# pathint/RankCompV3.jl

Measured on AMD Instinct MI355X. Metric: gene-pair·sample comparisons/sec at 20k genes × 1k samples, higher is better.
Workload: dtype u16

## Files before the change

rankcompv3.jl_amd/_ffi.py:

```python
from __future__ import annotations

import ctypes
import os
import subprocess
from typing import NamedTuple

import numpy as np

_HERE = os.path.dirname(os.path.abspath(__file__))
LIB_PATH = os.environ.get("REO_LIB_PATH") or os.path.join(_HERE, "libreo_hip.so")
CSRC = os.path.join(_HERE, "csrc")

REO_OK, REO_EINVAL, REO_EHIP, REO_ECOMM, REO_ENOMEM = 0, -1, -2, -3, -4
NTIMINGS = 12
CALL_BINS = 8192

SYMBOLS = [
    "reo_version", "reo_last_error", "reo_create", "reo_destroy", "reo_trim_memory", "reo_set_shard", "reo_set_allreduce", "reo_set_allgather",
    "reo_create_multi", "reo_comm_unique_id", "reo_comm_init_rank",
    "reo_set_matrix_f64", "reo_set_matrix_i64", "reo_set_matrix_dev_f64", "reo_set_matrix_dev_i64",
    "reo_set_matrix_f32", "reo_set_matrix_i32", "reo_set_matrix_dev_f32", "reo_set_matrix_dev_i32",
    "reo_set_matrix_rm_f64", "reo_set_matrix_rm_i64", "reo_set_matrix_rm_f32", "reo_set_matrix_rm_i32",
    "reo_set_matrix_csc_f64", "reo_set_matrix_csc_i64", "reo_set_matrix_csc_f32", "reo_set_matrix_csc_i32",
    "reo_set_groups", "reo_compute_thresholds", "reo_set_thresholds", "reo_get_thresholds", "reo_threshold",
# ... 837 lines not shown
    def get_matrix(self) -> np.ndarray:
        info = self.info()
        dt = {1: np.float64, 2: np.int64, 3: np.float32}.get(info["resident_dtype"])
        if dt is None:
            raise DimensionMismatch(REO_EINVAL, "no expression matrix set")
        out = np.zeros((info["G"], info["S"]), dtype=dt, order="F")
        check(self._L.reo_get_matrix(self._h, _ptr(out), out.nbytes))
        return out

    def set_profiling(self, on: bool) -> None:
        check(self._L.reo_set_profiling(self._h, 1 if on else 0))

    def reset_timings(self) -> None:
        check(self._L.reo_reset_timings(self._h))

    def timings(self) -> dict:
        ms = np.zeros(NTIMINGS, dtype=np.float64)
        check(self._L.reo_get_timings(self._h, _ptr(ms), NTIMINGS))
        return {"transform_ms": ms[0], "k1_ms": ms[1], "k2_ms": ms[2], "iter_ms": ms[3], "k3_ms": max(ms[3] - ms[2], 0.0), "k2_launches": int(ms[4]),
                "k1_launches": int(ms[5]), "exchange_ms": ms[6], "pseudobulk_ms": ms[7], "k2_full_ms": ms[8],
                "k2_full_launches": int(ms[9]), "k2_delta_ms": ms[10], "set_matrix_host_wall_ms": ms[11]}

    def info(self) -> dict:
        w = np.zeros(32, dtype=np.int64)
        check(self._L.reo_get_info(self._h, _ptr(w), 32))
        v = np.zeros(28, dtype=np.int64)
        v[:] = w[:28]
        return {"G": int(v[0]), "S": int(v[1]), "Gp": int(v[2]), "table_bytes": int(v[3]), "has_ties": int(v[4]),
                "tiles_owned": int(v[5]), "tiles_total": int(v[6]), "tile_i": int(v[7]), "chunk_j": int(v[8]),
                "chunks_per_panel": int(v[9]), "unit_h": int(v[10]), "sample_slots": int(v[11]),
                "shared_group_counts": int(v[12]), "group_count_bytes": int(v[13]), "transform_in_lds": int(v[14]), "xcc_local_histograms": int(v[15]),
                "cycle_period": int(v[16]), "cycle_found_at_pass": int(v[17]), "cycle_passes_skipped": int(v[18]), "upload_link_bytes": int(v[19]),
                "eager_range_launches": int(v[20]), "rowmajor_upload": int(v[21]),
                "csc_upload": int(v[22]), "csc_nnz": int(v[23]), "resident_dtype": int(v[24]),
                "k1_slot_order": int(v[25]), "k1_half_tiles_separated": int(v[26]), "csc_device": int(v[27]),
                "k1_unslot_form": int(w[28]), "contrast_treat": int(w[29]), "k1_slot_sides": int(w[30]),
                "masked_build": int(w[31])}
```

rankcompv3.jl_amd/csrc/api.hip:

```cpp
#include <execinfo.h>
#include <signal.h>
#include <unistd.h>

#include <ctime>
#include <algorithm>
#include <chrono>
#include <cmath>
#include <cstdarg>
#include <cstdio>
#include <cstdlib>
#include <cstring>

#include "reo_internal.h"
#include "contrast.h"
#include "masked_pairs.h"
#include "sample_counts.h"
#include "upload_csc.h"

#include <mutex>
#include <unordered_map>

namespace reo {

static thread_local std::string g_err;
// ... 217 lines not shown
    (void)!write(2, head, sizeof head - 1);
    void *frames[64];
    const int n = backtrace(frames, 64);
    backtrace_symbols_fd(frames, n, 2);
    sigaction(sig, &g_old_action[sig == SIGSEGV ? 0 : (sig == SIGBUS ? 1 : 2)], nullptr);
    raise(sig);
}

static void install_segv_backtrace()
{
    static bool done = false;
    if (done) return;
    done = true;
    void *warm[2];
    (void)backtrace(warm, 2);
    struct sigaction sa;
    memset(&sa, 0, sizeof sa);
    sa.sa_handler = segv_backtrace;
    sa.sa_flags = SA_NODEFER;
    sigaction(SIGSEGV, &sa, &g_old_action[0]);
    sigaction(SIGBUS, &sa, &g_old_action[1]);
    sigaction(SIGABRT, &sa, &g_old_action[2]);
}

static double wall_us()
{
    timespec ts;
    clock_gettime(CLOCK_MONOTONIC, &ts);
    return ts.tv_sec * 1e6 + ts.tv_nsec * 1e-3;
}

static void drop_ref_mask(reo_ctx *c, const char *why)
{
    c->ref_slot = -1;
    c->ref_gone = why;
}

int32_t wait_or_drop_table(reo_ctx *c)
{
    const hipError_t e = stream_wait(c);
    if (e == hipSuccess) return REO_OK;
    c->built_k = -1;
    c->table_complete = false;
    drop_ref_mask(c, "a kernel queued on this context failed and the class table was dropped");
    set_error("a kernel queued on this context failed: %s (the class table was dropped: call reo_build_pairs again)", hipGetErrorString(e));
    return REO_EHIP;
// ... 246 lines not shown
    c->sc_slot2col_uploaded = nullptr;
    REO_HIP_CHECK(hipMemcpyAsync(c->sc_slot2col.p, c->sc_slot2col_host.data(), map.size() * sizeof(int32_t), hipMemcpyHostToDevice, c->stream));
    c->sc_slot2col_uploaded = c->sc_slot2col.p;
    return REO_OK;
}

int32_t need_complete_table(reo_ctx *c)
{
    if (c->built_k < 0) { set_error("no class table: call reo_build_pairs first"); return REO_EINVAL; }
    if (!c->table_complete) {
        set_error("shard %d of %d holds only its own part of the class table: attach a communicator (reo_comm_init_rank) or an "
                  "exchange hook (reo_set_allgather, reo_set_allreduce) before reo_build_pairs", c->rank, c->world);
        return REO_ECOMM;
    }
    return REO_OK;
}

}

using namespace reo;

extern "C" {

int32_t reo_version(void) { return 1200; }

int32_t reo_trim_memory(void)
{
    std::vector<Block> all;
    {
        Pool &P = pool();
        std::lock_guard<std::mutex> lk(P.mu);
        all.swap(P.free_blocks);
        P.cached = 0;
    }
    int dev = 0;
    const bool have_dev = hipGetDevice(&dev) == hipSuccess;
    for (const Block &b : all) {
        if (!b.pinned) (void)hipSetDevice(b.device);
        raw_free(b.p, b.pinned);
    }
    {
        Handles &H = handles();
        std::lock_guard<std::mutex> lk(H.mu);
        for (int k = 0; k < 2; ++k) {
            for (auto &st : H.streams[k]) { (void)hipSetDevice(st.first); (void)hipStreamDestroy(st.second); }
            for (auto &ev : H.events[k]) { (void)hipSetDevice(ev.first); (void)hipEventDestroy(ev.second); }
            H.streams[k].clear(); H.events[k].clear();
// ... 31 lines not shown
    if (const char *e = getenv("REO_K1_WAVE")) c->k1_wave = (e[0] != '0');
    if (const char *e = getenv("REO_K1_HALF")) c->k1_half = (e[0] != '0');
    if (const char *e = getenv("REO_K1_SLOTS")) c->k1_slots = (e[0] != '0');
    if (const char *e = getenv("REO_K1_QUEUE")) c->k1_queue = (e[0] != '0');
    if (const char *e = getenv("REO_K1_UNSLOT")) { const int v = atoi(e); c->k1_unslot = (v == 8 || v == 4) ? v : (e[0] == '0' ? 0 : -1); }
    if (const char *e = getenv("REO_K1_SLOT_SIDES")) { const int v = atoi(e); c->k1_slot_sides = (v == 1 || v == 2) ? v : 0; }
    if (const char *e = getenv("REO_K1_WORKERS")) c->k1_workers = std::max(1, atoi(e));
    if (const char *e = getenv("REO_K1_ORDER")) c->k1_order = std::max(0, std::min(2, atoi(e)));
    {
        int n = 0;
        if (hipDeviceGetAttribute(&n, hipDeviceAttributeMultiprocessorCount, c->device) == hipSuccess && n > 0) c->n_cus = n;
    }
    if (const char *e = getenv("REO_SPIN_WAIT")) c->spin_wait = (e[0] != '0');
    if (const char *e = getenv("REO_CHECK_HOOK_TABLE")) c->check_hook_table = (e[0] != '0');
    if (const char *e = getenv("REO_SHARE_GROUP_COUNTS")) c->share_counts = (e[0] != '0');
    if (const char *e = getenv("REO_LIGHT_BAND")) c->light_band = std::max(0, atoi(e));
    if (const char *e = getenv("REO_HIST_BELOW")) c->hist_below = std::max(0, atoi(e));
    if (const char *e = getenv("REO_CYCLE")) c->cycle_watch = atoi(e) != 0;
    if (const char *e = getenv("REO_LIGHT")) c->light_mode = e[0] == '0' ? 0 : (e[0] == '2' ? 2 : (e[0] == '3' ? 3 : 1));
    c->light_window = light_window(); c->light_min_g = light_min_genes();
    if (const char *e = getenv("REO_LIGHT_WINDOW")) c->light_window = std::max(1, std::min(31, atoi(e)));
    if (const char *e = getenv("REO_LIGHT_MIN_G")) c->light_min_g = std::max(64, atoi(e));
    if (const char *e = getenv("REO_STATE_MIRROR")) c->state_mirror_wanted = (e[0] != '0');
    if (const char *e = getenv("REO_EXCHANGE_WAVES")) c->x_waves = std::max(1, std::min(8, atoi(e)));
    if (const char *e = getenv("REO_EAGER_UPLOAD")) c->eager_mode = std::max(0, std::min(2, atoi(e)));
    if (const char *e = getenv("REO_EAGER_CHUNK")) c->eager_chunk = std::max(1, atoi(e));
    if (const char *e = getenv("REO_EAGER_GATE")) c->eager_gate = atoi(e) != 0;
    if (const char *e = getenv("REO_EAGER_RANGES")) c->eager_ranges = std::max(1, std::min(6, atoi(e)));
    if (const char *e = getenv("REO_UPLOAD_THREADS")) c->upload_threads = std::max(0, std::min(64, atoi(e)));
    c->debug_passes = getenv("REO_DEBUG_PASSES") != nullptr;
    c->debug_stamps = getenv("REO_DEBUG_STAMPS") != nullptr;
    c->k1_stamps = getenv("REO_K1_STAMPS") != nullptr;
    hipError_t e = handle_stream(&c->stream, 0);
    if (e != hipSuccess) { delete c; set_error("hipStreamCreate failed: %s", hipGetErrorString(e)); return REO_EHIP; }
    int ok = 0;
    const char *xe = getenv("REO_XCC_LOCAL");
    if (!(xe && xe[0] == '0')) {
        const int32_t rc = xcc_selftest(c, &ok);
        if (rc) { reo_destroy(c); return rc; }
    }
    c->xcc_local = ok;
    *out = c;
    return REO_OK;
}

void reo_destroy(reo_ctx *c)
// ... 23 lines not shown
    for (auto &e : c->ev_rk) release_event(e, 0);
    for (auto &e : c->ev_up) release_event(e, 0);
    c->e_lists.release();
    for (int q = 0; q < 3; ++q) {
        if (c->stage_h[q]) pool_free(c->stage_h[q], c->stage_cap, true);
        c->stage_d[q].release();
        release_event(c->ev_stage[q], 0);
        release_event(c->ev_widen[q], 0);
    }
    release_event(c->ev_fork, 0);
    release_event(c->ev_x, 0);
    for (auto &e : c->ev_k1) release_event(e, 0);
    c->t_pos16.release(); c->t_lo16.release(); c->t_hi16.release(); c->gcounts.release();
    c->k1_slot_part.release(); c->k1_slot_maps.release(); c->pos_s.release(); c->lo_s.release(); c->k1_queue_ctr.release();
    c->t_pos32.release(); c->t_lo32.release(); c->t_hi32.release(); c->t_vin32.release(); c->t_vout32.release();
    for (int t = 0; t < 2; ++t) { c->refbits[t].release(); c->refbytes[t].release(); }
    c->raw.release(); c->delta_list.release(); c->cont.release(); c->result.release(); c->sorted_d.release(); c->sorted_p.release();
    c->rank_s.release(); c->rank_a.release(); c->scal.release(); c->blockmin.release();
    c->state.release(); c->trace.release(); c->modes.release(); c->cand.release(); c->hist.release(); c->mrank.release(); c->lstate.release(); c->clist.release(); c->olist.release(); c->units_all.release(); c->xsend.release(); c->xrecv.release(); c->check_flag.release(); c->gridbar.release(); c->chunk_v.release(); c->chunk_i.release(); c->part.release();
    if (c->host_state) pool_free(c->host_state, sizeof(IterState), true);
    if (c->host_flags) pool_free(c->host_flags, 8 * sizeof(int32_t), true);
    release_event(c->ev_flags, 0);
    if (c->host_ref) pool_free(c->host_ref, c->host_ref_cap, true);
    release_stream(c->stream, 0);
    delete c;
    tl_release_synced = false;
}

int32_t reo_set_shard(reo_ctx *c, int32_t rank, int32_t world)
{
    if (!c) { set_error("null context"); return REO_EINVAL; }
    if (world < 1 || rank < 0 || rank >= world) { set_error("bad shard %d of %d", rank, world); return REO_EINVAL; }
    if (!c->peers.empty()) { set_error("a multi-GPU context (reo_create_multi) shards by itself"); return REO_EINVAL; }
    c->rank = rank; c->world = world;
    c->built_k = -1;
    drop_ref_mask(c, "reo_set_shard dropped the class table that the last reo_identify_degs ran on");
    c->eager_k1 = false;
    c->gc_valid = false;
    c->table_complete = false;
    return REO_OK;
}

int32_t reo_set_allreduce(reo_ctx *c, reo_allreduce_fn fn, void *user)
{
    if (!c) { set_error("null context"); return REO_EINVAL; }
    c->ar = fn; c->ar_user = user;
// ... 573 lines not shown
        st.need_full = 1;
        st.raw_pass = -1;
        st.kstar = -1;
        st.cyc_period = -1;
        *c->host_state = st;
    }
    const bool watch = c->cycle_watch && c->light_mode != 0 && (c->light_mode == 1 || G > 65535) && G >= c->light_min_g && n_iter > 0;
    if (watch) {
        if ((rc = c->snap.ensure(2 * static_cast<size_t>(c->Gp)))) return rc;
        c->host_state->cyc_period = 0;
    }
    c->it_cycle_period = 0; c->it_cycle_at = 0; c->it_cycle_skipped = 0;
    DrainOnExit drain(c);
    if ((rc = launch_iter_init(c, c->host_ref, c->host_state))) return rc;
    c->it_pval_deg = pval_deg; c->it_padj_deg = padj_deg; c->it_n_iter = n_iter; c->it_n_conv = n_conv;
    c->it_a0 = static_cast<int>(a - 1); c->it_b0 = static_cast<int>(b - 1);
    c->k2_idx = 0;
    const int light_form = (G > 65535 && c->light_mode != 0) ? 1 : c->light_mode;
    c->it_light_form = light_form;
    c->state_mirror = light_form != 2 && c->state_mirror_wanted;
    bool small = G < c->light_min_g || c->light_mode == 0;
    c->it_no_light = false;
    int passes = 0, seen_need_full = 1, light_batches = 0, idle_light = 0, idle_any = 0;
    while (n_iter > 0) {
        const int remaining = n_iter - passes;
        const double w_loop = c->debug_passes ? wall_us() : 0.0;
        const int nfull = small ? std::min(8, remaining) : (seen_need_full ? std::min(passes == 0 ? 4 : 2, remaining) : 0);
        const int nlight = (small || seen_need_full) ? 0 : std::min(light_batches == 0 ? 32 : kLightBatch, remaining);
        if (nlight > 0) ++light_batches;
        tic(c, 3);
        for (int t = 0; t < nfull; ++t)
            if ((rc = launch_full_pass(c, false))) return rc;
        if (nlight > 0 && light_form == 2) {
            if ((rc = launch_light_persistent(c))) return rc;
        } else if (nlight > 0) {
            if ((rc = launch_light_batch(c, nlight))) return rc;
        }
        toc(c);
        if (!c->state_mirror) REO_HIP_CHECK(hipMemcpyAsync(c->host_state, c->state.p, sizeof(IterState), hipMemcpyDeviceToHost, c->stream));
        const double w0 = c->debug_passes ? wall_us() : 0.0;
        if ((rc = wait_or_drop_table(c))) return rc;
        if (c->debug_passes) fprintf(stderr, "  waited %.0f us for the batch (enqueueing it took %.0f us)\n", wall_us() - w0, w0 - w_loop);
        if (c->debug_passes && nlight > 0 && light_form == 3) {
            static LightState hs;
            if (hipMemcpy(&hs, c->lstate.p, sizeof hs, hipMemcpyDeviceToHost) == hipSuccess)
                for (int q = 1; q <= nlight; ++q)
                    if (hs.slot[q].pad0[0] || q <= 3)
                        fprintf(stderr, "  launch %d: why %d (1 window, 2 se left the bracket, 4 the histogram's cut left the band, 8 a list overflowed, 16 too many listed, 32 cut below the band), "
                                "cut of the m_lo histogram %d, listed %d, surely inside %d, cut %d (band around %d), eta %.3g, se %.10g\n", q, hs.slot[q].pad0[0], hs.slot[q].pad0[1],
                                hs.slot[q].pad0[2], hs.slot[q].pad0[3], hs.slot[q].pad0[4], hs.slot[q - 1].rec.kstar, hs.slot[q - 1].eta, hs.slot[q].se_base);
        }
        if (c->debug_passes)
            fprintf(stderr, "batch: %d sorting + %d light launches, passes %d -> %d, need_full %d, done %d, last_full %d, changed genes in front of the next pass %d\n", nfull, nlight,
                    passes, c->host_state->passes, c->host_state->need_full, c->host_state->done, c->host_state->last_full,
                    c->host_state->delta_cnt[c->host_state->passes & 1]);
        if ((rc = pass_fault(c))) return rc;
        idle_any = c->host_state->passes == passes ? idle_any + 1 : 0;
        if (idle_any >= 4) {
            set_error("the iteration made no progress in four batches of launches (passes %d, need_full %d): loop control fault", passes, c->host_state->need_full);
            return REO_EHIP;
        }
        if (nlight > 0) idle_light = c->host_state->passes == passes ? idle_light + 1 : 0;
        if (idle_light >= 2 && !small) {
            small = true;
            c->it_no_light = true;
        }
        if (c->host_state->passes < passes || c->host_state->passes > n_iter) {
            set_error("the iteration's pass counter reads %d after %d of %d passes: loop control fault", c->host_state->passes, passes, n_iter);
            return REO_EHIP;
        }
        passes = c->host_state->passes;
        seen_need_full = c->host_state->need_full;
        if (c->host_state->done || passes >= n_iter) break;
        if (c->host_state->cyc_period > 0) {
            const int p = c->host_state->cyc_period, P = (p & 1) ? 2 * p : p;
            const int skip = (n_iter - passes - 1) / P * P;
            if ((rc = launch_cycle_skip(c, skip, p))) return rc;
            c->it_cycle_period = p; c->it_cycle_at = passes; c->it_cycle_skipped = skip;
            if (c->debug_passes) fprintf(stderr, "cycle: the reference set in front of pass %d equals that of pass %d; %d passes skipped\n", passes, passes - p, skip);
            passes += skip;
        }
    }
    if (passes > 0 && !c->host_state->last_full) {
        tic(c, 3);
        if ((rc = launch_full_pass(c, true))) return rc;
        toc(c);
    }
    if (trace && passes > 0)
        REO_HIP_CHECK(hipMemcpyAsync(trace, c->trace.p, sizeof(int32_t) * 2 * passes, hipMemcpyDeviceToHost, c->stream));
    const int nk2 = std::min<int>(c->k2_idx, static_cast<int>(c->modes.n));
    if (c->profiling && nk2 > 0) {
        c->k2_modes.assign(c->k2_idx, 0);
        REO_HIP_CHECK(hipMemcpyAsync(c->k2_modes.data(), c->modes.p, sizeof(int32_t) * nk2, hipMemcpyDeviceToHost, c->stream));
    }
    if (c->debug_stamps) {
        unsigned long long st[24];
        REO_HIP_CHECK(hipMemcpy(st, c->scal.p + 32, sizeof st, hipMemcpyDeviceToHost));
        if (light_form == 3) {
            fprintf(stderr, "stamps kl_one (inputs back, se, cut, lists + mask step, changed rows, delta1, sums + windows, end):");
            for (int k = 0; k <= 7; ++k) fprintf(stderr, " %lld", (long long)(st[k] - st[8]));
        } else if (light_form == 2) {
            fprintf(stderr, "stamps kl_persist, one pass (phase 1, barrier, phase 2, barrier, loads asked, cut, mask step):");
            for (int k = 1; k <= 7; ++k) fprintf(stderr, " %lld", (long long)(st[k] - st[0]));
        } else {
            fprintf(stderr, "stamps kl_head (inputs back, cut, mask step, changed rows, delta1, window flags, block sums, end):");
            for (int k = 0; k <= 7; ++k) fprintf(stderr, " %lld", (long long)(st[k] - st[8]));
            fprintf(stderr, "\nstamps kl_rank (inputs back, selection + se, p + BH rank, end):");
            for (int k = 20; k <= 23; ++k) fprintf(stderr, " %lld", (long long)(st[k] - st[19]));
        }
        fprintf(stderr, "  (x 10 ns)\n");
    }
    if (iters_run) *iters_run = passes;
    const double w_copy = c->debug_passes ? wall_us() : 0.0;
    REO_HIP_CHECK(hipMemcpyAsync(result, c->result.p, sizeof(double) * 15 * G, hipMemcpyDeviceToHost, c->stream));
    const double w_copied = c->debug_passes ? wall_us() : 0.0;
    if ((rc = wait_or_drop_table(c))) return rc;
    drain.dismiss();
    if (c->debug_passes) fprintf(stderr, "  result copy: enqueued in %.0f us, waited %.0f us\n", w_copied - w_copy, wall_us() - w_copied);
    collect_timings(c);
    if ((rc = pass_fault(c))) return rc;
    if (passes > 0) c->ref_slot = (passes - 1) & 1;
    else drop_ref_mask(c, "the last reo_identify_degs was called with n_iter <= 0: no pass ran, no tallies were counted");
    return REO_OK;
}

int32_t reo_get_ref_mask(reo_ctx *c, uint8_t *ref_mask, int32_t *nref)
{
    int32_t rc = use(c);
    if (rc) return rc;
    if (!ref_mask) { set_error("reo_get_ref_mask: ref_mask must not be null"); return REO_EINVAL; }
    if (c->ref_slot < 0 || c->built_k < 0) {
        set_error("reo_get_ref_mask: no reference set to deliver: %s", c->ref_slot < 0 ? c->ref_gone : "the class table was dropped");
        return REO_EINVAL;
    }
    DrainOnExit drain(c);
    REO_HIP_CHECK(hipMemcpyAsync(ref_mask, c->refbytes[c->ref_slot].p, static_cast<size_t>(c->G), hipMemcpyDeviceToHost, c->stream));
    REO_HIP_CHECK(hipStreamSynchronize(c->stream));
    drain.dismiss();
    int32_t n = 0;
    for (int64_t i = 0; i < c->G; ++i) { ref_mask[i] = ref_mask[i] != 0; n += ref_mask[i]; }
    if (nref) *nref = n;
// ... 34 lines not shown
{
    if (!c) { set_error("null context"); return REO_EINVAL; }
    collect_timings(c);
    for (double &v : c->t_ms) v = 0.0;
    return REO_OK;
}

int32_t reo_get_timings(reo_ctx *c, double *ms, int32_t n)
{
    if (!c || !ms) { set_error("null argument"); return REO_EINVAL; }
    collect_timings(c);
    for (int i = 0; i < n && i < REO_NTIMINGS; ++i) ms[i] = c->t_ms[i];
    return REO_OK;
}

int32_t reo_get_info(reo_ctx *c, int64_t *info, int32_t n)
{
    if (!c || !info) { set_error("null argument"); return REO_EINVAL; }
    int64_t separated = 0;
    if (n > 26 && c->last_k1_slots) {
        int32_t rc = use(c);
        if (rc || (rc = launch_slot_separated(c, &separated))) return rc;
    }
    const int64_t v[32] = {c->G, c->S, c->Gp, static_cast<int64_t>(c->table.n * sizeof(uint32_t)), c->has_ties,
                           c->tiles_owned, c->tiles_total, kTileI, c->k1_cj, c->k1_q, kUnitH,
                           c->goff32.empty() ? 0 : c->goff32.back(), c->last_k1_shared,
                           static_cast<int64_t>(c->gcounts.n * sizeof(uint16_t)), c->transform_in_lds, c->xcc_local,
                           c->it_cycle_period, c->it_cycle_at, c->it_cycle_skipped, c->narrowed_bytes, c->eager_range_launches, c->rowmajor_upload,
                           c->csc_upload, c->csc_nnz, c->dtype, c->last_k1_slots, separated, c->csc_device,
                           c->last_k1_slots ? c->last_k1_unslot : 0, c->built_k >= 0 ? c->built_treat : -1,
                           c->last_k1_slots ? c->last_k1_slot_sides : 0, (c->built_k >= 0 && c->built_masked) ? 1 : 0};
    for (int i = 0; i < n && i < 32; ++i) info[i] = v[i];
    return REO_OK;
}

}
```

rankcompv3.jl_amd/csrc/kernels.hip:

```cpp
#include <algorithm>
#include <chrono>
#include <cstddef>
#include <cstdio>
#include <cstdlib>
#include <cstring>
#include <mutex>
#include <type_traits>

#include "reo_internal.h"
#include "k1_items.h"
#include "k1_slots.h"
#include "k1_queue.h"
#include "contrast.h"
#include "tie_coin.h"

namespace reo {

namespace {

template <bool COH, class T>
__device__ __forceinline__ T ldc(const T *p)
{
    if (COH) return __hip_atomic_load(p, __ATOMIC_RELAXED, __HIP_MEMORY_SCOPE_AGENT);
    return *p;
// ... 1505 lines not shown

struct IterArgs {
    IterState *st;
    const uint32_t *table;
    int G, Gp, Wp;
    int n_iter, n_conv;
    int a0, b0;
    double pval_deg, padj_deg;
    uint32_t *refbits[2];
    uint8_t *refbytes[2];
    int32_t *raw;
    uint32_t *delta_list;
    double *result;
    double *chunk_v; uint16_t *chunk_i; double *chunk_spl;
    double *sorted_d; double *sorted_spl; double *sorted_p;
    uint32_t *rank_s; uint32_t *rank_a;
    double *part; double *blockmin; double *scal;
    int32_t *trace; int32_t *modes;
    double *cand;
    int32_t *hist;
    int hist_stride;
    int32_t *mrank;
    int replay;
    int k2_idx;
    int xcc_local;
    int32_t *olist;
    int hist_below;
    uint8_t *snap;
    int32_t *clist; int band;
    int window, light_min_g;
    unsigned long long *stamps;
    IterState *host_st;
};

#ifdef REO_STAMPS
#define STAMP(a, k) do { if (blockIdx.x == 0 && threadIdx.x == 0) (a).stamps[k] = __builtin_amdgcn_s_memrealtime(); } while (0)
#else
#define STAMP(a, k) do { } while (0)
#endif

__device__ __forceinline__ void raise_fault(const IterArgs &a, int code)
{
    a.st->fault = code;
    if (a.host_st) a.host_st->fault = code;
}

constexpr int kCandMax = 64;
constexpr int kWindow = 24;
constexpr int kLightMinG = 4096;

__device__ __forceinline__ bool full_pass_active(const IterArgs &a, int &t, int &nref)
{
    const IterState *st = a.st;
    if (a.replay) { t = st->passes - 1; nref = st->nref_prev; return t >= 0; }
    t = st->passes; nref = st->nref;
    return !st->done && st->passes < a.n_iter && st->need_full;
}

__global__ __launch_bounds__(256) void k2_tally(IterArgs a)
{
    int t, nref;
    if (!full_pass_active(a, t, nref) || a.st->raw_pass == t) return;
    const int cur = t & 1;
    const int n = a.st->delta_cnt[cur];
    const bool full = n > kDeltaMax;
    if (a.modes && blockIdx.x == 0 && threadIdx.x == 0) a.modes[a.k2_idx] = full ? 1 : 0;
    if (full) tally_rows(reinterpret_cast<const uint4 *>(a.table), reinterpret_cast<const uint4 *>(a.refbits[cur]), a.G, a.Wp / 4, a.raw);
    else if (static_cast<int>(blockIdx.x) * 256 < a.G) delta_genes(a.table, a.G, a.Wp, a.delta_list + static_cast<size_t>(cur) * a.Gp, n, a.raw);
}

__global__ __launch_bounds__(256) void k2_scan(const uint32_t *__restrict__ table, const uint4 *__restrict__ refbits, int G, int Wp,
                                               int32_t *__restrict__ raw)
{
    tally_rows(reinterpret_cast<const uint4 *>(table), refbits, G, Wp / 4, raw);
}

// ... 427 lines not shown
    __shared__ double tail[kMaxBlocks + 1];
    const int nb = (G + 1023) / 1024;
    __shared__ double bm[kMaxBlocks];
    for (int b = threadIdx.x; b < nb; b += 256) bm[b] = a.blockmin[b];
    __syncthreads();
    for (int b = threadIdx.x; b <= nb; b += 256) {
        double run = INFINITY;
        for (int k = b + 1; k < nb; ++k) { const double m = bm[k]; run = m < run ? m : run; }
        tail[b] = run;
    }
    __syncthreads();
    const int i = blockIdx.x * 256 + threadIdx.x;
    bool ind = false, in_cut = false;
    if (i < G) {
        const uint32_t r = a.rank_a[i];
        double q = a.sorted_p[r];
        const double tl = tail[r >> 10];
        q = tl < q ? tl : q;
        q = q < 1.0 ? q : 1.0;
        a.result[static_cast<size_t>(G) + i] = q;
        in_cut = q <= a.padj_deg;
        ind = !(a.result[i] <= a.pval_deg && in_cut);
    }
    if (a.replay) return;
    const int over = publish_mask(a, t, i, ind, in_cut);
    if (over < 0) return;
    const int W = a.window;
    bool ok = G >= a.light_min_g && a.a0 - W >= 0 && a.b0 + W < G && a.a0 + W < a.b0 - W;
    if (ok) {
        const double va = a.sorted_d[a.a0], vb = a.sorted_d[a.b0];
        const double wa_lo = a.sorted_d[a.a0 - W], wa_hi = a.sorted_d[a.a0 + W];
        const double wb_lo = a.sorted_d[a.b0 - W], wb_hi = a.sorted_d[a.b0 + W];
        ok = wa_hi < wb_lo;
        a.scal[1] = wa_lo; a.scal[2] = wa_hi; a.scal[3] = wb_lo; a.scal[4] = wb_hi;
        a.scal[5] = va - wa_lo; a.scal[6] = wa_hi - va; a.scal[7] = vb - wb_lo; a.scal[8] = wb_hi - vb;
    }
    a.st->need_full = (over || !ok) ? 1 : 0;
    if (a.host_st) {
        IterState *h = a.host_st;
        h->passes = t + 1; h->done = a.st->done; h->need_full = (over || !ok) ? 1 : 0; h->last_full = 1;
        h->delta_cnt[(t + 1) & 1] = a.st->delta_cnt[(t + 1) & 1];
    }
}


template <int K, int J>
__device__ __forceinline__ void sort_stage(double &x, int t)
// ... 386 lines not shown
        const int4 *o = reinterpret_cast<const int4 *>(a.raw + static_cast<size_t>(i) * kRaw);
        r0 = o[0]; r1 = o[1];
    }
    if (b > 0) {
        const LightSlot *ps = &ls->slot[b - 1];
        r = ps->rec; bfail = ps->bfail; cdiff = ps->cdiff; cfound = ps->cfound;
#pragma unroll
        for (int q = 0; q < kSpread; ++q) { sig += ps->lc.sig[q][0]; nlow += ps->lc.nlow[q][0]; }
#pragma unroll
        for (int q = 0; q < 4; ++q) win[q] = ps->wnext[q];
    } else {
#pragma unroll
        for (int q = 0; q < 4; ++q) win[q] = a.scal[1 + q];
    }
    if (!TAIL) STAMP(a, 0);
    int n = 0;
    bool inref = false;
    bool stepped = false;
    if (b == 0) {
        const IterState *st = a.st;
        r.t = st->passes; r.nref = st->nref; r.nref_prev = st->nref_prev; r.done = st->done; r.need_full = st->need_full;
        r.raw_pass = st->raw_pass; r.ran = 0; r.dcnt = st->delta_cnt[r.t & 1]; r.kstar = -1;
        r.cper = st->cyc_period; r.cpow = st->cyc_pow; r.clam = st->cyc_lam; r.csel = st->cyc_sel; cdiff = st->cyc_ndiff;
        r.active = (!r.done && r.t < a.n_iter && !r.need_full) ? 1 : 0;
        if (r.active) {
            n = r.raw_pass == r.t ? 0 : min(r.dcnt, kDeltaMax);
            if (static_cast<int>(threadIdx.x) < n) dl[threadIdx.x] = a.delta_list[static_cast<size_t>(r.t & 1) * Gp + threadIdx.x];
            inref = i < G && a.refbytes[r.t & 1][i] != 0;
            lds_barrier();
        }
    } else if (r.active && bfail) {
        r.active = 0; r.need_full = 1;
    } else if (r.active && cfound) {
        r.active = 0; r.cper = cfound;
    } else if (r.active) {
        const int t = r.t, cur = t & 1, nxt = cur ^ 1;
        const int off = hist_first(r.kstar, a.hist_below), srel = sig - off;
        {
            const int32_t *hist = a.hist + static_cast<size_t>(pb) * kHistParts * a.hist_stride;
#pragma unroll
            for (int x = 0; x < kHistParts; ++x) {
                hv[0][0] += hx[x][0].x; hv[0][1] += hx[x][0].y; hv[0][2] += hx[x][0].z; hv[0][3] += hx[x][0].w;
                hv[0][4] += hx[x][1].x; hv[0][5] += hx[x][1].y; hv[0][6] += hx[x][1].z; hv[0][7] += hx[x][1].w;
            }
            if (srel > 2048) {
#pragma unroll 1
                for (int x = 0; x < kHistParts; ++x)
// ... 131 lines not shown
        if (blockIdx.x == 0 && wave == 0) {
            cyc_close();
            if (cfound) r.cper = cfound;
        }
        if (blockIdx.x == 0 && threadIdx.x == 0) {
            IterState *st = a.st;
            st->cyc_period = r.cper; st->cyc_pow = r.cpow; st->cyc_lam = r.clam; st->cyc_sel = r.csel; st->cyc_ndiff = cdiff;
            st->passes = r.t; st->nref = r.nref; st->nref_prev = r.nref_prev; st->done = r.done; st->need_full = r.need_full;
            st->i_iter = r.t - (r.done ? 1 : 0);
            st->raw_pass = r.raw_pass;
            st->delta_cnt[r.t & 1] = r.dcnt;
            if (r.ran) st->last_full = 0;
            if (stepped) { a.scal[1] = win[0]; a.scal[2] = win[1]; a.scal[3] = win[2]; a.scal[4] = win[3]; }
            if (a.host_st) {
                IterState *h = a.host_st;
                h->passes = r.t; h->done = r.done; h->need_full = r.need_full; h->delta_cnt[r.t & 1] = r.dcnt;
                h->cyc_period = r.cper;
                if (r.ran) h->last_full = 0;
            }
        }
        return;
    }
    if (r.active) r.raw_pass = r.t;
    if (blockIdx.x == 0 && threadIdx.x == 0) ls->slot[b].rec = r;
    if (!r.active || static_cast<int>(blockIdx.x) * 256 >= G) {
        if (blockIdx.x == 0 && wave == 0) { cyc_close(); if (lane == 0) { ls->slot[b].cdiff = cdiff; ls->slot[b].cfound = cfound; } }
        return;
    }
    const int pbuf = b & 1;
    LightCnt *lc = &ls->slot[b].lc;
    const double wa_lo = win[0], wa_hi = win[1], wb_lo = win[2], wb_hi = win[3];
    double v = 0.0;
    bool inner = false, inA = false, inB = false, belowA = false, belowB = false;
    if (n) {
        int d[kRaw];
        delta_counts_block(a.table, a.Wp, dl, n, d, dbuf);
        if (!TAIL) STAMP(a, 3);
        if (i < G) {
            r0.x += d[0]; r0.y += d[1]; r0.z += d[2]; r0.w += d[3];
            r1.x += d[4]; r1.y += d[5]; r1.z += d[6]; r1.w += d[7];
            int4 *o = reinterpret_cast<int4 *>(a.raw + static_cast<size_t>(i) * kRaw);
            o[0] = r0; o[1] = r1;
        }
    }
    if (i < G) {
        int32_t c[9];
        const bool tok = tallies_from(r0, r1, r.nref - (inref ? 1 : 0), c);
// ... 1489 lines not shown
    c->t_ms[4] += 1.0;
    k3_tallies<<<(G + 255) / 256, 256, 0, c->stream>>>(c->raw.p, c->refbytes[0].p, nref, G, c->cont.p);
    REO_HIP_CHECK(hipGetLastError());
    return REO_OK;
}

static IterArgs iter_args(reo_ctx *c, int replay)
{
    IterArgs a;
    a.st = c->state.p; a.table = c->table.p;
    a.G = static_cast<int>(c->G); a.Gp = c->Gp; a.Wp = c->Wp;
    a.n_iter = c->it_n_iter; a.n_conv = c->it_n_conv; a.a0 = c->it_a0; a.b0 = c->it_b0;
    a.pval_deg = c->it_pval_deg; a.padj_deg = c->it_padj_deg;
    for (int t = 0; t < 2; ++t) { a.refbits[t] = c->refbits[t].p; a.refbytes[t] = c->refbytes[t].p; }
    a.raw = c->raw.p; a.delta_list = c->delta_list.p; a.result = c->result.p;
    const int nchunk = (a.G + kSortChunk - 1) / kSortChunk;
    a.chunk_v = c->chunk_v.p; a.chunk_i = c->chunk_i.p;
    a.chunk_spl = c->chunk_v.p + static_cast<size_t>(nchunk) * kSortChunk;
    a.sorted_d = c->sorted_d.p; a.sorted_spl = c->sorted_d.p + ((c->G + 63) / 64) * 64;
    a.sorted_p = c->sorted_p.p; a.rank_s = c->rank_s.p; a.rank_a = c->rank_a.p;
    a.part = c->part.p; a.blockmin = c->blockmin.p; a.scal = c->scal.p;
    a.trace = c->trace.p; a.modes = nullptr;
    a.cand = c->cand.p; a.hist = c->hist.p; a.hist_stride = static_cast<int>(c->hist.n / (3 * kHistParts)); a.mrank = c->mrank.p;
    a.replay = replay; a.k2_idx = 0;
    a.clist = c->clist.p; a.olist = c->olist.p; a.band = c->light_band; a.hist_below = c->hist_below; a.snap = c->snap.p; a.xcc_local = c->xcc_local;
    a.window = c->light_window; a.light_min_g = (c->it_no_light || c->light_mode == 0) ? 0x7FFFFFFF : c->light_min_g;
    a.stamps = reinterpret_cast<unsigned long long *>(c->scal.p + 32);
    a.host_st = c->state_mirror ? c->host_state : nullptr;
    return a;
}

int32_t launch_full_pass(reo_ctx *c, bool replay)
{
    IterArgs a = iter_args(c, replay ? 1 : 0);
    const int G = a.G, nb = (G + 255) / 256;
    const int nchunk = (G + kSortChunk - 1) / kSortChunk;
    const int nmerge = (nchunk * kSortChunk + kMergeThreads / kMergeLanes - 1) / (kMergeThreads / kMergeLanes);
    if (!replay) {
        if (c->k2_idx < static_cast<int>(c->modes.n)) { a.modes = c->modes.p; a.k2_idx = c->k2_idx; }
        ++c->k2_idx;
        tic(c, 2);
        k2_tally<<<(G + 3) / 4, 256, 0, c->stream>>>(a);
        toc(c);
        c->t_ms[4] += 1.0;
    }
    k3_derive<<<nb, 256, 0, c->stream>>>(a);
    k3_sort_chunks<<<nchunk, kSortChunk, 0, c->stream>>>(a);
    const size_t spl_bytes = static_cast<size_t>(nchunk) * kSplit * sizeof(double);
    if (spl_bytes > (size_t(48) << 10))
        REO_HIP_CHECK(hipFuncSetAttribute(reinterpret_cast<const void *>(k3_merge_rank), hipFuncAttributeMaxDynamicSharedMemorySize, static_cast<int>(spl_bytes)));
    k3_merge_rank<<<nmerge, kMergeThreads, spl_bytes, c->stream>>>(a, nchunk);
    k3_abs_rank<<<nb, 256, static_cast<size_t>((G + 63) / 64) * sizeof(double), c->stream>>>(a, nmerge);
    k3_bh_local<<<(G + 1023) / 1024, 1024, 0, c->stream>>>(a);
    k3_finalize<<<c->Gp / 256, 256, 0, c->stream>>>(a);
    REO_HIP_CHECK(hipGetLastError());
    return REO_OK;
}

int32_t launch_light_persistent(reo_ctx *c)
{
    const IterArgs a = iter_args(c, 0);
    const unsigned nwg = static_cast<unsigned>(a.Gp / 256);
    REO_HIP_CHECK(hipMemsetAsync(c->gridbar.p, 0, sizeof(unsigned), c->stream));
    REO_HIP_CHECK(hipMemsetAsync(c->lstate.p, 0, 2 * sizeof(LightSlot), c->stream));
    kl_persist<<<nwg, 256, 0, c->stream>>>(a, c->lstate.p, c->gridbar.p);
    REO_HIP_CHECK(hipGetLastError());
    return REO_OK;
}

int32_t launch_light_batch(reo_ctx *c, int nlight)
{
    const IterArgs a = iter_args(c, 0);
    const int nb = (a.G + 255) / 256, nbp = a.Gp / 256;
    if (nlight < 1 || nlight > kLightBatch) { set_error("light batch of %d passes", nlight); return REO_EINVAL; }
    REO_HIP_CHECK(hipMemsetAsync(c->lstate.p, 0, static_cast<size_t>(nlight + 1) * sizeof(LightSlot), c->stream));
    if (c->it_light_form == 3) {
        REO_HIP_CHECK(hipMemsetAsync(c->hist.p, 0, static_cast<size_t>(kHistParts) * a.hist_stride * sizeof(int32_t), c->stream));
        for (int b = 0; b < nlight; ++b) kl_one<false><<<nbp, 256, 0, c->stream>>>(a, c->lstate.p, b);
        kl_one<true><<<nbp, 256, 0, c->stream>>>(a, c->lstate.p, nlight);
        REO_HIP_CHECK(hipGetLastError());
        return REO_OK;
    }
    for (int b = 0; b < nlight; ++b) {
        if (b < 2) kl_head<false, false><<<nbp, 256, 0, c->stream>>>(a, c->lstate.p, b);
        else kl_head<false, true><<<nbp, 256, 0, c->stream>>>(a, c->lstate.p, b);
        kl_rank<<<nb, 256, 0, c->stream>>>(a, c->lstate.p, b);
    }
    if (nlight < 2) kl_head<true, false><<<nbp, 256, 0, c->stream>>>(a, c->lstate.p, nlight);
    else kl_head<true, true><<<nbp, 256, 0, c->stream>>>(a, c->lstate.p, nlight);
    REO_HIP_CHECK(hipGetLastError());
    return REO_OK;
}

int32_t xcc_selftest(reo_ctx *c, int *ok)
{
// ... 44 lines not shown
```

rankcompv3.jl_amd/csrc/reo_internal.h:

```cpp
#pragma once

#include <hip/hip_runtime.h>

#include <cstdint>
#include <functional>
#include <string>
#include <vector>

#include "reo_hip.h"

namespace reo {

constexpr int kTileJ = 256;
constexpr int kTileI = 32;
constexpr int kPlanes = 4;
constexpr int kUnitH = 32;
constexpr int kRJ = 4;
constexpr int kRJTies = 2;
constexpr int kMaxGenes = 262143;
constexpr int kGenePad = 1024;
constexpr int kRaw = 8;
constexpr int kDeltaMax = 128;
constexpr int kSortChunk = 1024;

// ... 269 lines not shown
    reo::DevBuf<uint16_t> chunk_i;
    reo::DevBuf<double> part;
    reo::DevBuf<reo::IterState> state;
    reo::DevBuf<int32_t> trace;
    reo::DevBuf<int32_t> modes;
    reo::DevBuf<double> cand;
    reo::DevBuf<unsigned> gridbar;
    reo::DevBuf<reo::LightState> lstate;
    reo::DevBuf<int32_t> clist;
    int light_band = 32;
    bool cycle_watch = true;
    reo::DevBuf<uint8_t> snap;
    int it_cycle_period = 0, it_cycle_at = 0, it_cycle_skipped = 0;
    int hist_below = 256;
    int xcc_local = 0;
    int light_window = 24, light_min_g = 4096;
    int light_mode = 1;
    reo::DevBuf<int32_t> olist;
    reo::DevBuf<int32_t> hist, mrank;
    double it_pval_deg = 1.0, it_padj_deg = 0.05;
    int it_n_iter = 0, it_n_conv = 0, it_a0 = 0, it_b0 = 0;
    int k2_idx = 0;
    int it_light_form = 1;
    bool it_no_light = false;
    reo::IterState *host_state = nullptr;
    bool state_mirror_wanted = true;
    bool debug_passes = false, debug_stamps = false, k1_stamps = false;
    bool state_mirror = false;
    uint8_t *host_ref = nullptr;
    size_t host_ref_cap = 0;

    bool profiling = false;
    double t_ms[REO_NTIMINGS] = {0};
    std::vector<std::pair<int, reo::StageTimer>> pending;
    std::vector<reo::StageTimer> pool;
    std::vector<size_t> open;
    std::vector<int32_t> k2_modes;
    size_t k2_seen = 0;
};

namespace reo {

int32_t run_transform(reo_ctx *c);
enum { kLayoutColMajor = 0, kLayoutRowMajor = 1, kLayoutCsc = 2 };
int32_t eager_upload(reo_ctx *c, const void *hX, int64_t hld, bool with_k1, bool host_i32 = false, int layout = kLayoutColMajor);
int32_t upload_columns(reo_ctx *c, const void *hX, int64_t hld, int64_t G, int64_t ncols, void *dX, int dtype, int layout = kLayoutColMajor);
int32_t widen_device_i32(reo_ctx *c, const void *dX32, int64_t ld, int64_t G, int64_t S, void *dX64);
int32_t densify_device_csc(reo_ctx *c, int64_t G, int64_t S, const int64_t *colptr, const void *rows, int32_t index_bits, const void *vals,
                           int dtype, void *dX);
int32_t ensure_upload_streams(reo_ctx *c);
int32_t ensure_staging(reo_ctx *c, size_t slot_bytes);
void host_parallel(int nthreads, int ntasks, const std::function<void(int)> &fn);

struct K1Range { int b0, b1; bool first, last; };
int32_t launch_k1(reo_ctx *c, int k, int sides = 3, bool keep_table = false, const int32_t *gate = nullptr, const K1Range *range = nullptr,
                  bool prepare = false, int treat = -1);
int32_t k1_planes_fit(reo_ctx *c, bool *fit, size_t *need_bytes);
int64_t exchange_unit_words(const reo_ctx *c);
int32_t exchange_units_per_rank(const reo_ctx *c);
int32_t launch_pack_units(reo_ctx *c, int m0 = 0, int mcnt = -1, uint32_t *send = nullptr, hipStream_t st = nullptr);
int32_t launch_expand_units(reo_ctx *c, int m0 = 0, int mcnt = -1, const uint32_t *recv = nullptr, hipStream_t st = nullptr);
int32_t launch_slot_separated(reo_ctx *c, int64_t *half_tiles);
int32_t launch_counts(reo_ctx *c, int64_t i0, int64_t i1, int64_t j0, int64_t j1, uint16_t *d_gt, uint16_t *d_eq);
int32_t launch_check_table(reo_ctx *c, int *bad);
int32_t launch_decode(reo_ctx *c, int64_t i0, int64_t i1, int64_t j0, int64_t j1, uint8_t *d_code);
int32_t launch_pack_ref(reo_ctx *c, const uint8_t *d_bytes, uint32_t *d_bits);
int32_t launch_cycle_skip(reo_ctx *c, int skip, int period);
int32_t launch_iter_init(reo_ctx *c, const uint8_t *host_ref, const IterState *host_state);
int32_t launch_tally(reo_ctx *c, int nref);
int32_t launch_full_pass(reo_ctx *c, bool replay);
int32_t launch_light_persistent(reo_ctx *c);
int32_t launch_light_batch(reo_ctx *c, int nlight);
int32_t xcc_selftest(reo_ctx *c, int *ok);
int32_t light_min_genes();
int32_t light_window();
int32_t launch_mccullagh(reo_ctx *c, const int32_t *d_cont, int64_t n, double *d_out);

int32_t launch_pair_count(reo_ctx *c, const int32_t *d_genes, int64_t n_genes, const uint32_t *d_maskbits, uint32_t class_mask, int32_t *d_count);
int32_t launch_pair_fill(reo_ctx *c, const int32_t *d_genes, int64_t n_genes, const uint32_t *d_maskbits, uint32_t class_mask, const int64_t *d_rowptr,
                         int32_t *d_partner, uint8_t *d_code, int64_t capacity, int32_t *d_flag);

int plane_bits(int64_t G);
int32_t launch_sample_counts(reo_ctx *c, const int32_t *d_genes, int64_t n_queries, const uint32_t *d_maskbits, uint32_t class_mask,
                             const int32_t *d_slot2col, int32_t *d_sel, int32_t *d_gt, int32_t *d_eq);

int32_t launch_sample_fisher(reo_ctx *c, int64_t n_queries, const int32_t *d_sel_a, const int32_t *d_sel_b, const int32_t *d_gt_a,
                             const int32_t *d_eq_a, const int32_t *d_gt_b, const int32_t *d_eq_b, const double *d_lf, int64_t lf_entries,
                             int32_t *d_rev_up, int32_t *d_rev_down, int32_t *d_tied, double *d_p_up, double *d_p_down, int32_t *d_flag);

int32_t launch_call_rank(reo_ctx *c, int64_t n_genes, int64_t q0, int64_t nq, const double *d_p_up, const double *d_p_down, double pval_deg,
                         double padj_deg, uint32_t *d_words);
int32_t launch_call_cut(reo_ctx *c, int64_t n_genes, const uint32_t *d_words, int32_t *d_kstar, int32_t *d_cut, int32_t *d_n_up, int32_t *d_n_down);
int32_t launch_call_emit(reo_ctx *c, int64_t n_genes, const uint32_t *d_words, const int32_t *d_kstar, int8_t *d_calls);

struct PsItem;
// ... 54 lines not shown
```

Baseline: 51130 billion.

## Chain light iteration batches via device progress notify and gate closing replay on device

After: 51610 billion (median of 5 runs). About the same (+0.9%).

```diff
diff --git a/rankcompv3.jl_amd/_ffi.py b/rankcompv3.jl_amd/_ffi.py
--- a/rankcompv3.jl_amd/_ffi.py
+++ b/rankcompv3.jl_amd/_ffi.py
@@ -883,8 +883,8 @@
                 "k2_full_launches": int(ms[9]), "k2_delta_ms": ms[10], "set_matrix_host_wall_ms": ms[11]}
 
     def info(self) -> dict:
-        w = np.zeros(32, dtype=np.int64)
-        check(self._L.reo_get_info(self._h, _ptr(w), 32))
+        w = np.zeros(34, dtype=np.int64)
+        check(self._L.reo_get_info(self._h, _ptr(w), 34))
         v = np.zeros(28, dtype=np.int64)
         v[:] = w[:28]
         return {"G": int(v[0]), "S": int(v[1]), "Gp": int(v[2]), "table_bytes": int(v[3]), "has_ties": int(v[4]),
@@ -896,4 +896,4 @@
                 "csc_upload": int(v[22]), "csc_nnz": int(v[23]), "resident_dtype": int(v[24]),
                 "k1_slot_order": int(v[25]), "k1_half_tiles_separated": int(v[26]), "csc_device": int(v[27]),
                 "k1_unslot_form": int(w[28]), "contrast_treat": int(w[29]), "k1_slot_sides": int(w[30]),
-                "masked_build": int(w[31])}
+                "masked_build": int(w[31]), "chained_batches": int(w[32]), "gated_replay": int(w[33])}
diff --git a/rankcompv3.jl_amd/csrc/api.hip b/rankcompv3.jl_amd/csrc/api.hip
--- a/rankcompv3.jl_amd/csrc/api.hip
+++ b/rankcompv3.jl_amd/csrc/api.hip
@@ -263,6 +263,9 @@
     sigaction(SIGBUS, &sa, &g_old_action[1]);
     sigaction(SIGABRT, &sa, &g_old_action[2]);
 }
+
+static int light_notify_launch(int n) { return std::max(0, std::min(n - 1, (3 * n) / 4)); }
+constexpr double kChainQueryUs = 20.0;
 
 static double wall_us()
 {
@@ -555,7 +558,7 @@
 
 extern "C" {
 
-int32_t reo_version(void) { return 1200; }
+int32_t reo_version(void) { return 1300; }
 
 int32_t reo_trim_memory(void)
 {
@@ -633,6 +636,7 @@
     if (const char *e = getenv("REO_LIGHT_WINDOW")) c->light_window = std::max(1, std::min(31, atoi(e)));
     if (const char *e = getenv("REO_LIGHT_MIN_G")) c->light_min_g = std::max(64, atoi(e));
     if (const char *e = getenv("REO_STATE_MIRROR")) c->state_mirror_wanted = (e[0] != '0');
+    if (const char *e = getenv("REO_CHAIN")) c->chain = (e[0] != '0');
     if (const char *e = getenv("REO_EXCHANGE_WAVES")) c->x_waves = std::max(1, std::min(8, atoi(e)));
     if (const char *e = getenv("REO_EAGER_UPLOAD")) c->eager_mode = std::max(0, std::min(2, atoi(e)));
     if (const char *e = getenv("REO_EAGER_CHUNK")) c->eager_chunk = std::max(1, atoi(e));
@@ -702,6 +706,7 @@
     if (c->host_flags) pool_free(c->host_flags, 8 * sizeof(int32_t), true);
     release_event(c->ev_flags, 0);
     if (c->host_ref) pool_free(c->host_ref, c->host_ref_cap, true);
+    if (c->host_trace) pool_free(c->host_trace, c->host_trace_cap * sizeof(int32_t), true);
     release_stream(c->stream, 0);
     delete c;
     tl_release_synced = false;
@@ -1321,19 +1326,60 @@
     bool small = G < c->light_min_g || c->light_mode == 0;
     c->it_no_light = false;
     int passes = 0, seen_need_full = 1, light_batches = 0, idle_light = 0, idle_any = 0;
+    const bool chain_ok = c->chain && c->state_mirror && light_form == 1;
+    c->it_chained = 0; c->it_gated_replay = 0;
+    bool closed = false;
+    if (chain_ok && n_iter > 0 && c->host_trace_cap < 2 * static_cast<size_t>(n_iter)) {
+        if (c->host_trace) pool_free(c->host_trace, c->host_trace_cap * sizeof(int32_t), true);
+        c->host_trace = nullptr; c->host_trace_cap = 0;
+        REO_HIP_CHECK(pool_alloc(reinterpret_cast<void **>(&c->host_trace), 2 * static_cast<size_t>(n_iter) * sizeof(int32_t), true));
+        c->host_trace_cap = 2 * static_cast<size_t>(n_iter);
+    }
     while (n_iter > 0) {
         const int remaining = n_iter - passes;
         const double w_loop = c->debug_passes ? wall_us() : 0.0;
         const int nfull = small ? std::min(8, remaining) : (seen_need_full ? std::min(passes == 0 ? 4 : 2, remaining) : 0);
         const int nlight = (small || seen_need_full) ? 0 : std::min(light_batches == 0 ? 32 : kLightBatch, remaining);
         if (nlight > 0) ++light_batches;
+        bool closing = false;
         tic(c, 3);
         for (int t = 0; t < nfull; ++t)
-            if ((rc = launch_full_pass(c, false))) return rc;
+            if ((rc = launch_full_pass(c, 0))) return rc;
         if (nlight > 0 && light_form == 2) {
             if ((rc = launch_light_persistent(c))) return rc;
         } else if (nlight > 0) {
-            if ((rc = launch_light_batch(c, nlight))) return rc;
+            int start = passes, left = remaining, nl = nlight;
+            for (;;) {
+                const bool reaches = nl == left;
+                const int notify_b = (chain_ok && !reaches) ? light_notify_launch(nl) : -1;
+                const double w_b = c->debug_passes ? wall_us() : 0.0;
+                if ((rc = launch_light_batch(c, nl, notify_b))) return rc;
+                if (chain_ok && reaches) {
+                    if ((rc = launch_full_pass(c, 2))) return rc;
+                    REO_HIP_CHECK(hipMemcpyAsync(c->host_trace, c->trace.p, sizeof(int32_t) * 2 * n_iter, hipMemcpyDeviceToHost, c->stream));
+                    REO_HIP_CHECK(hipMemcpyAsync(result, c->result.p, sizeof(double) * 15 * G, hipMemcpyDeviceToHost, c->stream));
+                    closing = true;
+                }
+                if (c->debug_passes) fprintf(stderr, "  light batch of %d passes from pass %d%s: enqueued in %.0f us\n", nl, start, closing ? " with the closing sequence" : "", wall_us() - w_b);
+                if (notify_b < 0) break;
+                const volatile int32_t *progress = &c->host_state->pad[0];
+                bool alive = false;
+                double w_query = wall_us();
+                for (;;) {
+                    if (*progress >= start + notify_b) { alive = true; break; }
+                    const double w_now = wall_us();
+                    if (w_now - w_query < kChainQueryUs) continue;
+                    w_query = w_now;
+                    if (hipStreamQuery(c->stream) != hipErrorNotReady) {
+                        alive = *progress >= start + notify_b;
+                        break;
+                    }
+                }
+                if (!alive) break;
+                if (c->debug_passes) fprintf(stderr, "  pass %d reported %.0f us after the batch was enqueued: the next batch goes behind it\n", start + notify_b, wall_us() - w_b);
+                ++c->it_chained; ++light_batches;
+                start += nl; left -= nl; nl = std::min(kLightBatch, left);
+            }
         }
         toc(c);
         if (!c->state_mirror) REO_HIP_CHECK(hipMemcpyAsync(c->host_state, c->state.p, sizeof(IterState), hipMemcpyDeviceToHost, c->stream));
@@ -1349,10 +1395,12 @@
                                 "cut of the m_lo histogram %d, listed %d, surely inside %d, cut %d (band around %d), eta %.3g, se %.10g\n", q, hs.slot[q].pad0[0], hs.slot[q].pad0[1],
                                 hs.slot[q].pad0[2], hs.slot[q].pad0[3], hs.slot[q].pad0[4], hs.slot[q - 1].rec.kstar, hs.slot[q - 1].eta, hs.slot[q].se_base);
         }
-        if (c->debug_passes)
-            fprintf(stderr, "batch: %d sorting + %d light launches, passes %d -> %d, need_full %d, done %d, last_full %d, changed genes in front of the next pass %d\n", nfull, nlight,
-                    passes, c->host_state->passes, c->host_state->need_full, c->host_state->done, c->host_state->last_full,
-                    c->host_state->delta_cnt[c->host_state->passes & 1]);
+        if (c->debug_passes) {
+            const IterState *h = c->host_state;
+            const bool gated = closing && (h->done || h->passes >= n_iter) && h->last_full && h->cyc_period <= 0;
+            fprintf(stderr, "batch: %d sorting + %d light launches, passes %d -> %d, need_full %d, done %d, last_full %d, changed genes in front of the next pass %d%s\n", nfull, nlight,
+                    passes, h->passes, h->need_full, h->done, gated ? 0 : h->last_full, h->delta_cnt[h->passes & 1], gated ? " (the closing replay has run behind it)" : "");
+        }
         if ((rc = pass_fault(c))) return rc;
         idle_any = c->host_state->passes == passes ? idle_any + 1 : 0;
         if (idle_any >= 4) {
@@ -1370,7 +1418,10 @@
         }
         passes = c->host_state->passes;
         seen_need_full = c->host_state->need_full;
-        if (c->host_state->done || passes >= n_iter) break;
+        if (c->host_state->done || passes >= n_iter) {
+            if (closing && c->host_state->last_full && c->host_state->cyc_period <= 0) { closed = true; c->it_gated_replay = 1; }
+            break;
+        }
         if (c->host_state->cyc_period > 0) {
             const int p = c->host_state->cyc_period, P = (p & 1) ? 2 * p : p;
             const int skip = (n_iter - passes - 1) / P * P;
@@ -1382,11 +1433,13 @@
     }
     if (passes > 0 && !c->host_state->last_full) {
         tic(c, 3);
-        if ((rc = launch_full_pass(c, true))) return rc;
+        if ((rc = launch_full_pass(c, 1))) return rc;
         toc(c);
     }
-    if (trace && passes > 0)
-        REO_HIP_CHECK(hipMemcpyAsync(trace, c->trace.p, sizeof(int32_t) * 2 * passes, hipMemcpyDeviceToHost, c->stream));
+    if (trace && passes > 0) {
+        if (closed) memcpy(trace, c->host_trace, sizeof(int32_t) * 2 * passes);
+        else REO_HIP_CHECK(hipMemcpyAsync(trace, c->trace.p, sizeof(int32_t) * 2 * passes, hipMemcpyDeviceToHost, c->stream));
+    }
     const int nk2 = std::min<int>(c->k2_idx, static_cast<int>(c->modes.n));
     if (c->profiling && nk2 > 0) {
         c->k2_modes.assign(c->k2_idx, 0);
@@ -1411,11 +1464,16 @@
     }
     if (iters_run) *iters_run = passes;
     const double w_copy = c->debug_passes ? wall_us() : 0.0;
-    REO_HIP_CHECK(hipMemcpyAsync(result, c->result.p, sizeof(double) * 15 * G, hipMemcpyDeviceToHost, c->stream));
+    if (!closed) REO_HIP_CHECK(hipMemcpyAsync(result, c->result.p, sizeof(double) * 15 * G, hipMemcpyDeviceToHost, c->stream));
     const double w_copied = c->debug_passes ? wall_us() : 0.0;
-    if ((rc = wait_or_drop_table(c))) return rc;
+    if (!closed || (c->profiling && nk2 > 0)) {
+        if ((rc = wait_or_drop_table(c))) return rc;
+    }
     drain.dismiss();
-    if (c->debug_passes) fprintf(stderr, "  result copy: enqueued in %.0f us, waited %.0f us\n", w_copied - w_copy, wall_us() - w_copied);
+    if (c->debug_passes) {
+        if (closed) fprintf(stderr, "  result and trace arrived behind the last batch (%d batches chained, closing replay gated on the device)\n", c->it_chained);
+        else fprintf(stderr, "  result copy: enqueued in %.0f us, waited %.0f us\n", w_copied - w_copy, wall_us() - w_copied);
+    }
     collect_timings(c);
     if ((rc = pass_fault(c))) return rc;
     if (passes > 0) c->ref_slot = (passes - 1) & 1;
@@ -1496,16 +1554,17 @@
         int32_t rc = use(c);
         if (rc || (rc = launch_slot_separated(c, &separated))) return rc;
     }
-    const int64_t v[32] = {c->G, c->S, c->Gp, static_cast<int64_t>(c->table.n * sizeof(uint32_t)), c->has_ties,
+    const int64_t v[34] = {c->G, c->S, c->Gp, static_cast<int64_t>(c->table.n * sizeof(uint32_t)), c->has_ties,
                            c->tiles_owned, c->tiles_total, kTileI, c->k1_cj, c->k1_q, kUnitH,
                            c->goff32.empty() ? 0 : c->goff32.back(), c->last_k1_shared,
                            static_cast<int64_t>(c->gcounts.n * sizeof(uint16_t)), c->transform_in_lds, c->xcc_local,
                            c->it_cycle_period, c->it_cycle_at, c->it_cycle_skipped, c->narrowed_bytes, c->eager_range_launches, c->rowmajor_upload,
                            c->csc_upload, c->csc_nnz, c->dtype, c->last_k1_slots, separated, c->csc_device,
                            c->last_k1_slots ? c->last_k1_unslot : 0, c->built_k >= 0 ? c->built_treat : -1,
-                           c->last_k1_slots ? c->last_k1_slot_sides : 0, (c->built_k >= 0 && c->built_masked) ? 1 : 0};
-    for (int i = 0; i < n && i < 32; ++i) info[i] = v[i];
-    return REO_OK;
-}
-
-}
+                           c->last_k1_slots ? c->last_k1_slot_sides : 0, (c->built_k >= 0 && c->built_masked) ? 1 : 0,
+                           c->it_chained, c->it_gated_replay};
+    for (int i = 0; i < n && i < 34; ++i) info[i] = v[i];
+    return REO_OK;
+}
+
+}
diff --git a/rankcompv3.jl_amd/csrc/kernels.hip b/rankcompv3.jl_amd/csrc/kernels.hip
--- a/rankcompv3.jl_amd/csrc/kernels.hip
+++ b/rankcompv3.jl_amd/csrc/kernels.hip
@@ -1551,6 +1551,7 @@
     int hist_stride;
     int32_t *mrank;
     int replay;
+    int notify_b;
     int k2_idx;
     int xcc_local;
     int32_t *olist;
@@ -1581,6 +1582,10 @@
 __device__ __forceinline__ bool full_pass_active(const IterArgs &a, int &t, int &nref)
 {
     const IterState *st = a.st;
+    if (a.replay == 2) {
+        t = st->passes - 1; nref = st->nref_prev;
+        return t >= 0 && (st->done || st->passes >= a.n_iter) && !st->last_full && st->cyc_period <= 0;
+    }
     if (a.replay) { t = st->passes - 1; nref = st->nref_prev; return t >= 0; }
     t = st->passes; nref = st->nref;
     return !st->done && st->passes < a.n_iter && st->need_full;
@@ -2054,7 +2059,17 @@
         in_cut = q <= a.padj_deg;
         ind = !(a.result[i] <= a.pval_deg && in_cut);
     }
-    if (a.replay) return;
+    if (a.replay) {
+        if (a.replay == 2 && threadIdx.x == 0) {
+            __threadfence();
+            if (atomicAdd(&a.st->ticket, 1) == static_cast<int>(gridDim.x) - 1) {
+                a.st->ticket = 0;
+                a.st->last_full = 1;
+                if (a.host_st) a.host_st->last_full = 1;
+            }
+        }
+        return;
+    }
     const int over = publish_mask(a, t, i, ind, in_cut);
     if (over < 0) return;
     const int W = a.window;
@@ -2487,7 +2502,7 @@
         r.t = st->passes; r.nref = st->nref; r.nref_prev = st->nref_prev; r.done = st->done; r.need_full = st->need_full;
         r.raw_pass = st->raw_pass; r.ran = 0; r.dcnt = st->delta_cnt[r.t & 1]; r.kstar = -1;
         r.cper = st->cyc_period; r.cpow = st->cyc_pow; r.clam = st->cyc_lam; r.csel = st->cyc_sel; cdiff = st->cyc_ndiff;
-        r.active = (!r.done && r.t < a.n_iter && !r.need_full) ? 1 : 0;
+        r.active = (!r.done && r.t < a.n_iter && !r.need_full && r.cper <= 0) ? 1 : 0;
         if (r.active) {
             n = r.raw_pass == r.t ? 0 : min(r.dcnt, kDeltaMax);
             if (static_cast<int>(threadIdx.x) < n) dl[threadIdx.x] = a.delta_list[static_cast<size_t>(r.t & 1) * Gp + threadIdx.x];
@@ -2665,7 +2680,10 @@
         return;
     }
     if (r.active) r.raw_pass = r.t;
-    if (blockIdx.x == 0 && threadIdx.x == 0) ls->slot[b].rec = r;
+    if (blockIdx.x == 0 && threadIdx.x == 0) {
+        ls->slot[b].rec = r;
+        if (b == a.notify_b && r.active && a.host_st) a.host_st->pad[0] = r.t;
+    }
     if (!r.active || static_cast<int>(blockIdx.x) * 256 >= G) {
         if (blockIdx.x == 0 && wave == 0) { cyc_close(); if (lane == 0) { ls->slot[b].cdiff = cdiff; ls->slot[b].cfound = cfound; } }
         return;
@@ -4201,7 +4219,7 @@
     a.part = c->part.p; a.blockmin = c->blockmin.p; a.scal = c->scal.p;
     a.trace = c->trace.p; a.modes = nullptr;
     a.cand = c->cand.p; a.hist = c->hist.p; a.hist_stride = static_cast<int>(c->hist.n / (3 * kHistParts)); a.mrank = c->mrank.p;
-    a.replay = replay; a.k2_idx = 0;
+    a.replay = replay; a.k2_idx = 0; a.notify_b = -1;
     a.clist = c->clist.p; a.olist = c->olist.p; a.band = c->light_band; a.hist_below = c->hist_below; a.snap = c->snap.p; a.xcc_local = c->xcc_local;
     a.window = c->light_window; a.light_min_g = (c->it_no_light || c->light_mode == 0) ? 0x7FFFFFFF : c->light_min_g;
     a.stamps = reinterpret_cast<unsigned long long *>(c->scal.p + 32);
@@ -4209,9 +4227,9 @@
     return a;
 }
 
-int32_t launch_full_pass(reo_ctx *c, bool replay)
-{
-    IterArgs a = iter_args(c, replay ? 1 : 0);
+int32_t launch_full_pass(reo_ctx *c, int replay)
+{
+    IterArgs a = iter_args(c, replay);
     const int G = a.G, nb = (G + 255) / 256;
     const int nchunk = (G + kSortChunk - 1) / kSortChunk;
     const int nmerge = (nchunk * kSortChunk + kMergeThreads / kMergeLanes - 1) / (kMergeThreads / kMergeLanes);
@@ -4247,9 +4265,10 @@
     return REO_OK;
 }
 
-int32_t launch_light_batch(reo_ctx *c, int nlight)
-{
-    const IterArgs a = iter_args(c, 0);
+int32_t launch_light_batch(reo_ctx *c, int nlight, int notify_b)
+{
+    IterArgs a = iter_args(c, 0);
+    a.notify_b = c->it_light_form == 1 ? notify_b : -1;
     const int nb = (a.G + 255) / 256, nbp = a.Gp / 256;
     if (nlight < 1 || nlight > kLightBatch) { set_error("light batch of %d passes", nlight); return REO_EINVAL; }
     REO_HIP_CHECK(hipMemsetAsync(c->lstate.p, 0, static_cast<size_t>(nlight + 1) * sizeof(LightSlot), c->stream));
diff --git a/rankcompv3.jl_amd/csrc/reo_internal.h b/rankcompv3.jl_amd/csrc/reo_internal.h
--- a/rankcompv3.jl_amd/csrc/reo_internal.h
+++ b/rankcompv3.jl_amd/csrc/reo_internal.h
@@ -315,11 +315,15 @@
     int it_n_iter = 0, it_n_conv = 0, it_a0 = 0, it_b0 = 0;
     int k2_idx = 0;
     int it_light_form = 1;
+    int it_chained = 0, it_gated_replay = 0;
     bool it_no_light = false;
     reo::IterState *host_state = nullptr;
     bool state_mirror_wanted = true;
     bool debug_passes = false, debug_stamps = false, k1_stamps = false;
     bool state_mirror = false;
+    int chain = 1;
+    int32_t *host_trace = nullptr;
+    size_t host_trace_cap = 0;
     uint8_t *host_ref = nullptr;
     size_t host_ref_cap = 0;
 
@@ -361,9 +365,9 @@
 int32_t launch_cycle_skip(reo_ctx *c, int skip, int period);
 int32_t launch_iter_init(reo_ctx *c, const uint8_t *host_ref, const IterState *host_state);
 int32_t launch_tally(reo_ctx *c, int nref);
-int32_t launch_full_pass(reo_ctx *c, bool replay);
+int32_t launch_full_pass(reo_ctx *c, int replay);
 int32_t launch_light_persistent(reo_ctx *c);
-int32_t launch_light_batch(reo_ctx *c, int nlight);
+int32_t launch_light_batch(reo_ctx *c, int nlight, int notify_b = -1);
 int32_t xcc_selftest(reo_ctx *c, int *ok);
 int32_t light_min_genes();
 int32_t light_window();
```
